# gnns4hri/3D_multi_pose_estimator

Hardware: AMD Instinct MI355X
Metric: frames/sec (5-view Panoptic, 4 persons) at 1/2/4/8 GPUs; MPJPE vs ref (higher is better)
Workload: dtype f32

## Files before the change

3d_multi_pose_estimator_amd/csrc/api.hip:

```cpp
#include <cmath>
#include <cstdarg>
#include <new>
#include <cstdio>
#include <cstdlib>
#include <cstring>

#include "mpe_internal.h"

using namespace mpe;

namespace {

int fail(mpe_ctx *ctx, int code, const char *fmt, ...) {
    char buf[512];
    va_list ap;
    va_start(ap, fmt);
    vsnprintf(buf, sizeof buf, fmt, ap);
    va_end(ap);
    if (ctx) ctx->err = buf;
    return code;
}

#define HIPCHK(ctx, expr)                                                                     \
    do {                                                                                      \
// ... 467 lines not shown
        if (g.in_dim > 512) return false;
    }
    const size_t shm = (size_t)2 * ((size_t)16 * (ctx->cfg.max_heads_per_frame + 1) + (ctx->cfg.max_heads_per_frame + 1) + 1 +
                                    (size_t)(ctx->cfg.n_cameras + 1) * (ctx->cfg.n_cameras + 1)) * sizeof(float);
    return shm <= 40 * 1024;
}

int ensure_lat_workspace(mpe_ctx *ctx) {
    if (ctx->gat_pl[0]) return MPE_OK;
    ctx->lat_rows = ctx->max_nodes < LAT_MAX_NODES ? ctx->max_nodes : LAT_MAX_NODES;
    ctx->gat_pl_plane = (size_t)ctx->lat_rows * ctx->act_ld;
    int rc;
    for (int i = 0; i < 2; ++i)
        if ((rc = dev_alloc(ctx, &ctx->gat_pl[i], 3 * ctx->gat_pl_plane))) return rc;
    return MPE_OK;
}

struct LatTail {
    bool deferred = false;
    const float *ft2 = nullptr;
    int ld = 0;
    float alpha = 0.f, out_slope = 0.f;
    int out_mode = 0;
};

int run_gat_lat(mpe_ctx *ctx, hipStream_t s, const mpe_batch *b, float *d_scores_en, float *d_scores_heads, LatTail *tail = nullptr) {
    if (tail) tail->deferred = false;
    int rc = ensure_lat_workspace(ctx);
    if (rc) return rc;
    const int V = ctx->cfg.n_cameras, J = ctx->cfg.n_joints, hmax = ctx->cfg.max_heads_per_frame;
    const int n_nodes = b->n_heads + b->n_edge_nodes;
    if (n_nodes > ctx->lat_rows) return fail(ctx, MPE_ERR_CAPACITY, "latency path: %d nodes exceed %d", n_nodes, ctx->lat_rows);
    GatLayer &g0 = ctx->gat[0];
    uint16_t *head_src = getenv("MPE_NO_HEAD_SRC_TABLE") ? nullptr : ctx->head_src;
    {
        GemmProf gp(ctx, s, 2.0 * b->n_heads * (double)g0.in_dim * (J * 10), 0, 0);
        HIPCHK(ctx, launch_lat_l0a(s, ctx->d_cfg, *b, V, J, ctx->node_off, ctx->head_frame, ctx->en_frame, ctx->en_pair, ctx->head_src, hmax,
                                   ctx->d_status, ctx->l0_w, (long)weight_rows(g0.in_dim) * ctx->l0_ld, ctx->l0_ld, ctx->l0_b, g0.in_dim, ctx->h0,
                                   ctx->feat_ld, ctx->gat_alpha));
    }
    bool done = false;
    if ((rc = gat_linear(ctx, s, ctx->h0, ctx->feat_ld, g0.fc2, ctx->act[1], ctx->act_ld, b->n_heads, nullptr, false, 0.f, false, nullptr, nullptr,
                         -1.0, nullptr, &done)))
        return rc;
    const int L = ctx->gat_layers;
    for (int l = 0; l < L; ++l) {
// ... 41 lines not shown
            a.ld_out = 1;
            if (tail && coef && !d_scores_heads && g.heads == 1 && g.out_dim == 1) {
                tail->deferred = true;
                tail->ft2 = a.ft2;
                tail->ld = a.ld;
                tail->alpha = a.alpha;
                tail->out_slope = a.out_slope;
                tail->out_mode = a.out_mode;
                return MPE_OK;
            }
        } else {
            a.out_mode = 0;
            a.out = nullptr;
            a.out_pl = ctx->gat_pl[0];
            a.out_pl_plane = ctx->gat_pl_plane;
            a.ld_out = ctx->act_ld;
        }
        HIPCHK(ctx, launch_lat_attention(s, *b, V, hmax, ctx->node_off, ctx->head_frame, ctx->en_frame, ctx->en_pair, a, head_src));
    }
    return MPE_OK;
}

int run_gat(mpe_ctx *ctx, hipStream_t s, const mpe_batch *b, float *d_scores_en, float *d_scores_heads,
            const float *d_feats = nullptr, int ld_feats = 0) {
    int rc = ensure_gat_workspace(ctx);
    if (rc) return rc;
    if (lat_gat_ok(ctx, b, d_feats != nullptr)) return run_gat_lat(ctx, s, b, d_scores_en, d_scores_heads);
    const int V = ctx->cfg.n_cameras, J = ctx->cfg.n_joints;
    const int n_nodes = b->n_heads + b->n_edge_nodes;
    if ((rc = gat_topology(ctx, s, b))) return rc;
    const bool dense_in = d_feats != nullptr;
    if (dense_in) {
        if (ld_feats < ctx->gat[0].in_dim) return fail(ctx, MPE_ERR_INVALID, "feature stride too small");
        if (!ctx->xdense) {
            int rc2 = dev_alloc(ctx, &ctx->xdense, (size_t)ctx->max_nodes * ctx->feat_ld);
            if (rc2) return rc2;
            if ((rc2 = dev_alloc(ctx, &ctx->hdense, (size_t)ctx->max_nodes * ctx->feat_ld))) return rc2;
        }
        HIPCHK(ctx, hipMemcpy2DAsync(ctx->xdense, (size_t)ctx->feat_ld * sizeof(float), d_feats,
                                     (size_t)ld_feats * sizeof(float), (size_t)ctx->gat[0].in_dim * sizeof(float),
                                     n_nodes, hipMemcpyDeviceToDevice, s));
    } else if (ctx->l0_grouped) {
        HIPCHK(ctx, launch_head_features(s, ctx->d_cfg, *b, J, ctx->xc, ctx->l0_ld, 0, 0, false, ctx->cam_count, V));
        HIPCHK(ctx, launch_group_heads(s, b->n_heads, V, b->d_head_cam, ctx->cam_count, ctx->cam_list,
                                       ctx->cfg.max_heads, true));
    } else {
        HIPCHK(ctx, launch_head_features(s, ctx->d_cfg, *b, J, ctx->x0, ctx->feat_ld, 0, 0, true));
    }
    const int L = ctx->gat_layers;
    for (int l = 0; l < L; ++l) {
        const bool last = l == L - 1;
        AggArgs a = gat_agg_args(ctx, l);
        int n_rows_ft2 = 0;
        if ((rc = gat_layer_linear(ctx, s, b, l, l > 0 ? GAT_IN_ACT : dense_in ? GAT_IN_DENSE0 : GAT_IN_IMPLICIT, &a,
                                   &n_rows_ft2)))
            return rc;
        if (last) {
            a.out_mode = ctx->gat_out_mode;
            a.score_mode = 1;
            a.out = d_scores_en;
            a.out_heads = d_scores_heads;
            a.ld_out = 1;
        } else {
            a.out_mode = 0;
            a.out = ctx->act[0];
            a.ld_out = ctx->act_ld;
        }
        if ((rc = gat_attention(ctx, s, b, l, a, n_rows_ft2))) return rc;
    }
    return MPE_OK;
}

int copy_rows_in(mpe_ctx *ctx, hipStream_t s, float *dst, int ld_dst, const float *src, int ld_src, int cols, int rows) {
    if (rows <= 0) return MPE_OK;
    HIPCHK(ctx, hipMemsetAsync(dst, 0, (size_t)rows * ld_dst * sizeof(float), s));
    HIPCHK(ctx, hipMemcpy2DAsync(dst, (size_t)ld_dst * sizeof(float), src, (size_t)ld_src * sizeof(float),
                                 (size_t)cols * sizeof(float), rows, hipMemcpyDeviceToDevice, s));
    return MPE_OK;
}

}

extern "C" {

const char *mpe_version(void) { return "mpe-hip 0.1 (gfx950)"; }
// ... 419 lines not shown
    if ((rc = ensure_gat_workspace(ctx))) return rc;
    for (int k = 0; k < 2; ++k)
        if (ctx->pair_key[k] == b->d_xy) ctx->pair_key[k] = nullptr;
    if (lat_gat_ok(ctx, b, false) && lat_tail_available(hmax, ctx->cl_keys_per_frame) && b->n_edge_nodes > 0) {
        LatTail tail;
        if ((rc = run_gat_lat(ctx, s, b, scores, nullptr, &tail))) return rc;
        if (tail.deferred) {
            const int J = ctx->cfg.n_joints;
            const int slot = ctx->pair_next;
            const size_t need = (size_t)LAT_MAX_FRAMES * hmax * hmax * J * 3;
            const bool pairs_ok = (size_t)b->n_heads <= (size_t)LAT_MAX_FRAMES * hmax;
            if (pairs_ok && !ctx->pair_pts[slot] && (rc = dev_alloc(ctx, &ctx->pair_pts[slot], need, false))) return rc;
            for (int k = 0; k < 2; ++k)
                if (k == slot || ctx->pair_key[k] == b->d_xy) ctx->pair_key[k] = nullptr;
            HIPCHK(ctx, launch_lat_tail(s, ctx->d_cfg, *b, J, ctx->en_pair, ctx->en_frame, tail.ft2, tail.ld, ctx->a12, tail.alpha, tail.out_slope,
                                        tail.out_mode, ctx->node_off, scores, ctx->cfg.max_persons_per_frame, hmax, ctx->cl_keys_per_frame, d_persons,
                                        d_n_persons, pairs_ok ? ctx->pair_pts[slot] : nullptr));
            if (pairs_ok) {
                ctx->pair_key[slot] = b->d_xy;
                ctx->pair_heads[slot] = b->n_heads;
                ctx->pair_en[slot] = b->n_edge_nodes;
                ctx->pair_next = slot ^ 1;
            }
            return MPE_OK;
        }
    } else if ((rc = run_gat(ctx, s, b, scores, nullptr))) {
        return rc;
    }
    HIPCHK(ctx, launch_cluster(s, ctx->d_cfg, *b, ctx->en_pair, scores, ctx->cfg.max_persons_per_frame,
                               ctx->cfg.max_heads_per_frame, ctx->cl_keys, ctx->cl_keys_per_frame, ctx->cl_scratch,
                               ctx->cl_scratch_per_frame, d_persons, d_n_persons));
    return MPE_OK;
}

int mpe_mlp_input_rows(mpe_ctx *ctx, void *stream, const mpe_batch *b, const int32_t *d_persons,
                       const int32_t *d_n_persons, float *d_rows, int32_t ld_rows, uint8_t *d_valid) {
    int rc = check_batch(ctx, b);
    if (rc) return rc;
    if (b->n_frames == 0) return MPE_OK;
    DeviceGuard dg(ctx);
    const int width = ctx->cfg.n_cameras * ctx->cfg.n_joints * ctx->cfg.numbers_per_joint;
    if (!d_persons || !d_n_persons || !d_rows || ld_rows < width)
        return fail(ctx, MPE_ERR_INVALID, "mpe_mlp_input_rows: bad argument");
    HIPCHK(ctx, launch_mlp_rows(static_cast<hipStream_t>(stream), ctx->d_cfg, ctx->cfg.n_cameras, ctx->cfg.n_joints, *b,
                                d_persons, d_n_persons, nullptr, ctx->cfg.max_persons_per_frame, d_rows, ld_rows,
                                d_valid));
    return MPE_OK;
}

static int mlp_chain(mpe_ctx *ctx, hipStream_t s, const float *x, int ld_x, int m, const int32_t *d_m, float **y_out,
                     int *ld_y, const DecodeEpi *dec = nullptr, bool *dec_done = nullptr) {
    if (dec_done) *dec_done = false;
    const float *in = x;
    int ld_in = ld_x;
    int rc;
    for (int l = 0; l < ctx->mlp_layers; ++l) {
// ... 286 lines not shown
```

3d_multi_pose_estimator_amd/csrc/cluster.hip:

```cpp
#include <cstdlib>
#include <cstring>

#include "mpe_internal.h"
#include "dlt_common.h"

namespace mpe {

namespace {

struct PySet {
    int32_t *tab;
    int32_t *alt;
    int mask, fill;
};

__device__ inline int pyset_probe(const int32_t *tab, int mask, int key, bool stop_on_equal, bool *found) {
    unsigned perturb = (unsigned)key;
    int i = key & mask;
    *found = false;
    while (true) {
        int probes = (i + 9 <= mask) ? 9 : 0;
        int j = i;
        while (true) {
            const int cur = tab[j];
// ... 291 lines not shown
            for (int t = lane; t < n / 2; t += 64) {
                const int i = ((t & ~(j - 1)) << 1) | (t & (j - 1));
                const int p = i | j;
                const bool up = (i & k) == 0;
                const uint64_t x = s_keys[i], y = s_keys[p];
                if ((x > y) == up) {
                    s_keys[i] = y;
                    s_keys[p] = x;
                }
            }
            __syncthreads();
        }
    if (lane != 0) return;
    Work w = carve(s_work, hmax, table_cap);
    auto pair_of = [&](int m, int &h1, int &h2) {
        const uint32_t pr = s_pair[m];
        h1 = (int)(pr >> 16);
        h2 = (int)(pr & 0xFFFFu);
    };
    n_persons[f] = greedy_and_components(w, s_keys, n, pair_of, H, M, s_cam, V, cfg->min_views, pcap, out);
}

#define MPE_RL(v, i) __builtin_amdgcn_readlane((int)(v), (i))
__device__ inline int wl(int old, int val, int idx) { return (int)threadIdx.x == idx ? val : old; }

struct RegSet {
    int t0, t1;
    int mask, fill;
};

__device__ inline int rs_get(const RegSet &s, int j) { return j < 64 ? MPE_RL(s.t0, j) : MPE_RL(s.t1, j - 64); }

__device__ inline void rs_put(RegSet &s, int j, int key) {
    if (j < 64) s.t0 = wl(s.t0, key, j);
    else s.t1 = wl(s.t1, key, j - 64);
}

__device__ inline int rs_probe(const RegSet &s, int key, bool stop_on_equal, bool *found) {
    unsigned perturb = (unsigned)key;
    int i = key & s.mask;
    *found = false;
    while (true) {
        int probes = (i + 9 <= s.mask) ? 9 : 0;
        int j = i;
        while (true) {
            const int cur = rs_get(s, j);
            if (cur == -1) return j;
// ... 16 lines not shown
    if (found) return false;
    rs_put(s, j, key);
    s.fill++;
    if (s.fill * 5 < s.mask * 3) return true;
    const int minused = s.fill * 4;
    int newsize = 8;
    while (newsize <= minused) newsize <<= 1;
    RegSet n{-1, -1, newsize - 1, s.fill};
    for (int half = 0; half < 2; ++half) {
        const int t = half ? s.t1 : s.t0;
        unsigned long long bits = __ballot(t != -1);
        while (bits) {
            const int i = __builtin_ctzll(bits);
            bits &= bits - 1;
            bool f2;
            const int k = MPE_RL(t, i);
            rs_put(n, rs_probe(n, k, false, &f2), k);
        }
    }
    s = n;
    return true;
}

__device__ __forceinline__ void cluster_wave_body(uint64_t *s_keys, int f, const DevCfg *__restrict__ cfg, int n_frames,
                                                  const int32_t *__restrict__ head_off, const int32_t *__restrict__ en_off,
                                                  const int32_t *__restrict__ head_cam, const int32_t *__restrict__ en_pair,
                                                  const float *__restrict__ scores, int pcap, int n_pow2, int hmax,
                                                  int32_t *__restrict__ persons, int32_t *__restrict__ n_persons) {
    if (f >= n_frames) return;
    const int V = cfg->V;
    const int lane = threadIdx.x;
    const int h0 = head_off[f], H = head_off[f + 1] - h0;
    const int e0 = en_off[f], M = en_off[f + 1] - e0;
    int32_t *out = persons + (size_t)f * pcap * V;
    if (M <= 0 || H > 64 || H > hmax || M > n_pow2) {
        for (int i = lane; i < pcap * V; i += 64) out[i] = -1;
        if (lane == 0) n_persons[f] = 0;
        return;
    }
    uint32_t *s_pair = reinterpret_cast<uint32_t *>(s_keys + n_pow2);
    const float thr = cfg->threshold;
    const int min_views = cfg->min_views;
    int n_valid = 0;
    for (int m0 = 0; m0 < M; m0 += 64) {
        const int m = m0 + lane;
        uint64_t key = KEY_NONE;
        if (m < M) {
            const int h1 = en_pair[2 * (size_t)(e0 + m)], h2 = en_pair[2 * (size_t)(e0 + m) + 1];
            s_pair[m] = ((uint32_t)h1 << 16) | (uint32_t)h2;
            key = make_key(scores[e0 + m], thr, m);
        }
        const unsigned long long live = __ballot(key != KEY_NONE);
        if (key != KEY_NONE) s_keys[n_valid + __popcll(live & ((1ull << lane) - 1ull))] = key;
        n_valid += __popcll(live);
    }
    int n = 64;
    while (n < n_valid) n <<= 1;
    for (int m = n_valid + lane; m < n; m += 64) s_keys[m] = KEY_NONE;
    __syncthreads();
    for (int k = 2; k <= n; k <<= 1)
        for (int j = k >> 1; j > 0; j >>= 1) {
            for (int t = lane; t < n / 2; t += 64) {
                const int i = ((t & ~(j - 1)) << 1) | (t & (j - 1));
                const int p = i | j;
                const bool up = (i & k) == 0;
                const uint64_t x = s_keys[i], y = s_keys[p];
                if ((x > y) == up) {
                    s_keys[i] = y;
                    s_keys[p] = x;
                }
            }
            __syncthreads();
        }

    int32_t *s_aux = reinterpret_cast<int32_t *>(s_pair + n_pow2);
    int32_t *s_first = s_aux, *s_ord = s_aux + 64, *s_gor = s_aux + 128, *s_gcnt = s_aux + 192;
    const int camv = lane < H ? head_cam[h0 + lane] : 0;
    int linkedv = (int)(1u << camv);
    int humanv = -1, cfhv = 0, eav = -1, ebv = -1;

    s_first[lane] = 0x7FFFFFFF;
    s_gor[lane] = 0;
    s_gcnt[lane] = 0;
    __syncthreads();
    for (int m = lane; m < M; m += 64) {
        const uint32_t pr = s_pair[m];
        atomicMin(&s_first[pr >> 16], 2 * m);
        atomicMin(&s_first[pr & 0xFFFFu], 2 * m + 1);
    }
    __syncthreads();
    const int firstv = s_first[lane];
    const int n_nodes = __popcll(__ballot(firstv != 0x7FFFFFFF));
    {
        int rank = 0;
        for (int l = 0; l < H; ++l) rank += MPE_RL(firstv, l) < firstv ? 1 : 0;
        if (firstv != 0x7FFFFFFF) s_ord[rank] = lane;
    }
    __syncthreads();
    const int orderv = lane < n_nodes ? s_ord[lane] : 0;

    int cur = 0, ne = 0;
    for (int k0 = 0; k0 < n; k0 += 64) {
        const uint64_t key = s_keys[k0 + lane];
        const bool valid = key != KEY_NONE;
        const uint32_t pr = valid ? s_pair[(uint32_t)key] : 0u;
        const int h1 = (int)(pr >> 16), h2 = (int)(pr & 0xFFFFu);
        const bool first1 = pair_first_is_h1(h1, h2);
        const int a_l = first1 ? h1 : h2, b_l = first1 ? h2 : h1;
        const uint32_t ba_l = 1u << __shfl(camv, a_l), bb_l = 1u << __shfl(camv, b_l);
        const int cnt = __popcll(__ballot(valid));
        int start = 0;
        while (true) {
            const uint32_t la_l = (uint32_t)__shfl(linkedv, a_l), lb_l = (uint32_t)__shfl(linkedv, b_l);
            const int ha_l = __shfl(humanv, a_l), hb_l = __shfl(humanv, b_l);
            const uint32_t ca_x = (uint32_t)__shfl(cfhv, ha_l >= 0 ? ha_l : 0);
            const uint32_t cb_x = (uint32_t)__shfl(cfhv, hb_l >= 0 ? hb_l : 0);
            const uint32_t ca_l = ha_l >= 0 ? ca_x : 0u, cb_l = hb_l >= 0 ? cb_x : 0u;
            const bool rej = (lb_l & ba_l) || (la_l & bb_l) || (ca_l & bb_l) || (cb_l & ba_l) ||
                             (ha_l >= 0 && hb_l >= 0 && (cb_l & ca_l));
            const unsigned long long pass = __ballot(valid && lane >= start && !rej);
            if (!pass) break;
// ... 13 lines not shown
                cfhv = wl(cfhv, (int)(ca | bb), ha);
            } else if (hb >= 0 && ha < 0) {
                humanv = wl(humanv, hb, a);
                cfhv = wl(cfhv, (int)(cb | ba), hb);
            } else {
                humanv = humanv == hb ? ha : humanv;
            }
            eav = wl(eav, a, ne);
            ebv = wl(ebv, b, ne);
            ++ne;
            linkedv = wl(linkedv, (int)(la | bb), a);
            linkedv = wl(linkedv, (int)(lb | ba), b);
            start = q + 1;
        }
        if (cnt < 64) break;
    }

    if (humanv >= 0) {
        atomicOr(&s_gor[humanv], 1 << camv);
        atomicAdd(&s_gcnt[humanv], 1);
    }
    for (int i = lane; i < pcap * V; i += 64) out[i] = -1;
    __threadfence_block();
    __syncthreads();
    const bool plainv = __popc((unsigned)s_gor[lane]) == s_gcnt[lane];
    unsigned long long done = 0;
    int np = 0;
    for (int oi = 0; oi < n_nodes; ++oi) {
        const int v = MPE_RL(orderv, oi);
        if ((done >> v) & 1ull) continue;
        const int g = MPE_RL(humanv, v);
        if (g < 0 || MPE_RL((int)plainv, g)) {
            const unsigned long long memb = g >= 0 ? __ballot(humanv == g) : (1ull << v);
            done |= memb;
            if (__popcll(memb) >= min_views && np < pcap) {
                if ((memb >> lane) & 1ull) out[(size_t)np * V + camv] = lane;
                ++np;
            }
            continue;
        }
        RegSet set{-1, -1, 7, 0};
        rs_add(set, v);
        int lvlv = 0, nxtv = 0;
        lvlv = wl(lvlv, v, 0);
        int nl = 1;
        bool full = set.fill == n_nodes;
        while (nl > 0 && !full) {
// ... 39 lines not shown
    if (lane == 0) n_persons[f] = np;
}

__global__ __launch_bounds__(64) void k_cluster_wave(const DevCfg *__restrict__ cfg, int n_frames,
                                                     const int32_t *__restrict__ head_off,
                                                     const int32_t *__restrict__ en_off,
                                                     const int32_t *__restrict__ head_cam,
                                                     const int32_t *__restrict__ en_pair,
                                                     const float *__restrict__ scores, int pcap, int n_pow2,
                                                     int hmax, int32_t *__restrict__ persons,
                                                     int32_t *__restrict__ n_persons) {
    extern __shared__ uint64_t s_keys[];
    cluster_wave_body(s_keys, blockIdx.x, cfg, n_frames, head_off, en_off, head_cam, en_pair, scores, pcap, n_pow2, hmax, persons, n_persons);
}

struct TailScores {
    const float *ft2;
    int ld;
    const float *a12;
    float alpha, out_slope;
    int out_mode;
    const int32_t *node_off;
    float *scores;
};

__global__ __launch_bounds__(256) void k_lat_tail(const DevCfg *__restrict__ cfg, int n_frames, int n_en, int J,
                                                  const int32_t *__restrict__ head_off, const int32_t *__restrict__ en_off,
                                                  const int32_t *__restrict__ head_cam, const int32_t *__restrict__ en_pair,
                                                  const int32_t *__restrict__ en_frame, TailScores ts, int pcap, int n_pow2, int hmax,
                                                  int32_t *__restrict__ persons, int32_t *__restrict__ n_persons,
                                                  const uint32_t *__restrict__ tri_mask, const double *__restrict__ xy,
                                                  double *__restrict__ pair_pts) {
#pragma clang fp contract(off)
    extern __shared__ uint64_t s_keys[];
    if ((int)blockIdx.x < n_frames) {
        if (threadIdx.x >= 64) return;
        const int f = blockIdx.x, lane = threadIdx.x;
        const int hb = head_off[f], H = head_off[f + 1] - hb;
        const int e0 = en_off[f], M = en_off[f + 1] - e0;
        const int nb = ts.node_off[f];
        for (int m = lane; m < M; m += 64) {
            const int h1 = en_pair[2 * (size_t)(e0 + m)], h2 = en_pair[2 * (size_t)(e0 + m) + 1], v = H + m;
            const float *ra1 = ts.a12 + (size_t)(nb + h1) * 32, *ra2 = ts.a12 + (size_t)(nb + h2) * 32, *ra3 = ts.a12 + (size_t)(nb + v) * 32;
            const float a2v = ra3[16];
            float e1 = ra1[0] + a2v, e2 = ra2[0] + a2v, e3 = ra3[0] + a2v;
            e1 = e1 > 0.f ? e1 : e1 * ts.alpha;
            e2 = e2 > 0.f ? e2 : e2 * ts.alpha;
            e3 = e3 > 0.f ? e3 : e3 * ts.alpha;
            const float mx = fmaxf(fmaxf(e1, e2), e3);
            const float x1 = expf(e1 - mx), x2 = expf(e2 - mx), x3 = expf(e3 - mx);
            const float sum = (x1 + x2) + x3;
            const float w1 = x1 / sum, w2 = x2 / sum, w3 = x3 / sum;
            const float v1 = ts.ft2[(size_t)(nb + h1) * ts.ld], v2 = ts.ft2[(size_t)(nb + h2) * ts.ld], v3 = ts.ft2[(size_t)(nb + v) * ts.ld];
            float acc = v1 * w1;
            acc = acc + v2 * w2;
            acc = acc + v3 * w3;
            float o = acc;
            if (ts.out_mode == 0) o = acc > 0.f ? acc : acc * ts.out_slope;
            else if (ts.out_mode == 1) o = 1.f / (1.f + expf(-acc));
            ts.scores[e0 + m] = H > hmax ? 0.f : o;
        }
        __syncthreads();
        cluster_wave_body(s_keys, f, cfg, n_frames, head_off, en_off, head_cam, en_pair, ts.scores, pcap, n_pow2, hmax, persons, n_persons);
        return;
    }
    const size_t i = (size_t)(blockIdx.x - n_frames) * 256 + threadIdx.x;
    if (i >= (size_t)n_en * J) return;
    const int m = (int)(i / J), j = (int)(i - (size_t)m * J);
    const int f = en_frame[m];
    const int hb = head_off[f], H = head_off[f + 1] - hb;
    if (H > hmax) return;
    int la = en_pair[2 * (size_t)m], lb = en_pair[2 * (size_t)m + 1];
    int ca = head_cam[hb + la], cb = head_cam[hb + lb];
    if (ca > cb) {
        const int t = la;
        la = lb;
        lb = t;
        const int c = ca;
        ca = cb;
        cb = c;
    }
    const int ga = hb + la, gb = hb + lb;
    if (!((tri_mask[ga] >> j) & 1u) || !((tri_mask[gb] >> j) & 1u)) return;
    double ua, va, ub, vb;
    dltc::undistort_point(cfg, ca, xy[((size_t)ga * J + j) * 2], xy[((size_t)ga * J + j) * 2 + 1], &ua, &va);
    dltc::undistort_point(cfg, cb, xy[((size_t)gb * J + j) * 2], xy[((size_t)gb * J + j) * 2 + 1], &ub, &vb);
    dltc::dlt_solve(cfg->P[ca], cfg->P[cb], ua, va, ub, vb, pair_pts + (((size_t)ga * hmax + lb) * J + j) * 3);
}

bool lat_tail_available(int hmax, size_t keys_per_frame) {
    if (getenv("MPE_CLUSTER_KERNEL") || hmax > 64) return false;
    int n_pow2 = 64;
    while ((size_t)n_pow2 < keys_per_frame) n_pow2 <<= 1;
    return (size_t)n_pow2 * (sizeof(uint64_t) + sizeof(uint32_t)) + 256 * sizeof(int32_t) <= 48 * 1024;
}

hipError_t launch_lat_tail(hipStream_t s, const DevCfg *cfg, const mpe_batch &b, int J, const int32_t *en_pair, const int32_t *en_frame,
                           const float *ft2, int ld, const float *a12, float alpha, float out_slope, int out_mode, const int32_t *node_off,
                           float *scores, int pcap, int hmax, size_t keys_per_frame, int32_t *persons, int32_t *n_persons, double *pair_pts) {
    if (b.n_frames <= 0) return hipSuccess;
    int n_pow2 = 64;
    while ((size_t)n_pow2 < keys_per_frame) n_pow2 <<= 1;
    const size_t shm = (size_t)n_pow2 * (sizeof(uint64_t) + sizeof(uint32_t)) + 256 * sizeof(int32_t);
    TailScores ts{ft2, ld, a12, alpha, out_slope, out_mode, node_off, scores};
    const size_t items = pair_pts ? (size_t)b.n_edge_nodes * J : 0;
    const unsigned grid = (unsigned)(b.n_frames + (items + 255) / 256);
    hipLaunchKernelGGL(k_lat_tail, dim3(grid), dim3(256), shm, s, cfg, b.n_frames, pair_pts ? b.n_edge_nodes : 0, J, b.d_frame_head_off,
                       b.d_frame_en_off, b.d_head_cam, en_pair, en_frame, ts, pcap, n_pow2, hmax, persons, n_persons, b.d_tri_mask, b.d_xy,
                       pair_pts);
    return hipGetLastError();
}

constexpr int CB_THREADS = 1024;
constexpr int CB_WAVES = CB_THREADS / 64;
constexpr int CB_KCAP = 8192;
constexpr int CB_INF = 0x7FFFFFFF;

__global__ __launch_bounds__(CB_THREADS) void k_cluster_block(const DevCfg *__restrict__ cfg, int n_frames,
                                                              const int32_t *__restrict__ head_off,
                                                              const int32_t *__restrict__ en_off,
                                                              const int32_t *__restrict__ head_cam,
                                                              const int32_t *__restrict__ en_pair,
                                                              const float *__restrict__ scores, int pcap, int hmax,
                                                              int table_cap, uint64_t *__restrict__ keys_all,
                                                              size_t keys_per_frame, int32_t *__restrict__ persons,
                                                              int32_t *__restrict__ n_persons) {
    extern __shared__ uint64_t s_keys[];
    const int f = blockIdx.x;
    if (f >= n_frames) return;
    const int V = cfg->V;
    const int t = threadIdx.x, lane = t & 63, wave = t >> 6;
    const int h0 = head_off[f], H = head_off[f + 1] - h0;
// ... 322 lines not shown
```

3d_multi_pose_estimator_amd/csrc/mpe_internal.h:

```cpp
#pragma once
#include <hip/hip_runtime.h>
#include <stdint.h>
#include <string>
#include <vector>

#include "../../include/mpe.h"

namespace mpe {

constexpr int GEMM_BM = 128;
constexpr int GEMM_BN = 80;
constexpr int GEMM_BK = 32;
constexpr int GEMM_BN_MAX = 208;
inline int weight_rows(int out_dim) { return (out_dim + 15) / 16 * 16 + GEMM_BN_MAX; }
constexpr int LD_ALIGN = 32;

inline int round_up(int x, int m) { return (x + m - 1) / m * m; }

struct Linear {
    float *w = nullptr;
    float *b = nullptr;
    unsigned short *w16 = nullptr;
    int ldw16 = 0;
    unsigned short *w3 = nullptr;
// ... 81 lines not shown
    bool gat_split = true;
    mpe::Linear mlp[MPE_MAX_MLP_LAYERS];
    bool mlp_ready[MPE_MAX_MLP_LAYERS] = {};
    int max_nodes = 0;
    int feat_ld = 0;
    int act_ld = 0;
    float *x0 = nullptr;
    float *h0 = nullptr;
    float *xdense = nullptr;
    float *hdense = nullptr;
    float *xc = nullptr;
    int l0_ld = 0;
    mpe::Linear l0_fc1[MPE_MAX_CAMERAS];
    float *l0_w = nullptr;
    float *l0_b = nullptr;
    int32_t *cam_count = nullptr;
    int32_t *cam_list = nullptr;
    bool l0_grouped = true;
    float *act[3] = {nullptr, nullptr, nullptr};
    float *a12 = nullptr;
    double *pair_pts[2] = {nullptr, nullptr};
    const void *pair_key[2] = {nullptr, nullptr};
    int pair_heads[2] = {0, 0}, pair_en[2] = {0, 0}, pair_next = 0;
    unsigned short *gat_pl[2] = {nullptr, nullptr};
    size_t gat_pl_plane = 0;
    int lat_rows = 0;
    int32_t *head_frame = nullptr;
    int32_t *en_frame = nullptr;
    int32_t *en_pair = nullptr;
    uint16_t *head_src = nullptr;
    size_t head_src_cap = 0;
    int x_m_cap = 0;
    int32_t *node_off = nullptr;
    mpe::ResidualState *res_state = nullptr;
    uint32_t *res_hist = nullptr;
    double *res_partial = nullptr;
    double *log_table = nullptr;
    int n_log = 0;
    uint64_t *cl_keys = nullptr;
    int32_t *cl_scratch = nullptr;
    size_t cl_keys_per_frame = 0, cl_scratch_per_frame = 0;
    int mlp_ld_in = 0, mlp_ld_hidden = 0;
    float *mlp_rows = nullptr;
    float *mlp_act[2] = {nullptr, nullptr};
    int32_t *mlp_count = nullptr;
    float *scores_tmp = nullptr;
// ... 99 lines not shown
                          int32_t *en_frame, int32_t *en_pair, uint16_t *head_src, int hmax, int32_t *status, const float *l0_w,
                          long w_cam_stride, int l0_ld, const float *l0_b, int n_out, float *h0, int ld_h0, float alpha);
hipError_t launch_lat_attention(hipStream_t s, const mpe_batch &b, int V, int max_heads_per_frame, const int32_t *node_off,
                                const int32_t *head_frame, const int32_t *en_frame, const int32_t *en_pair, const AggArgs &a,
                                const uint16_t *head_src);
hipError_t launch_gat_attention(hipStream_t s, const mpe_batch &b, int V, int max_heads_per_frame,
                                const int32_t *node_off, const int32_t *head_frame, const int32_t *en_frame,
                                const int32_t *en_pair, const float *attn_l, const float *attn_r, float *a12,
                                const AggArgs &a, int n_rows_ft2, const uint16_t *head_src, int x_deg_cap = 0,
                                int x_m_cap = 0);

size_t cluster_keys_per_frame(int max_heads_per_frame);
size_t cluster_scratch_per_frame(int max_heads_per_frame);
hipError_t launch_cluster(hipStream_t s, const DevCfg *cfg, const mpe_batch &b, const int32_t *en_pair,
                          const float *scores, int pcap, int max_heads_per_frame, uint64_t *keys,
                          size_t keys_per_frame, int32_t *scratch, size_t scratch_per_frame,
                          int32_t *persons, int32_t *n_persons);

bool lat_tail_available(int hmax, size_t keys_per_frame);
hipError_t launch_lat_tail(hipStream_t s, const DevCfg *cfg, const mpe_batch &b, int J, const int32_t *en_pair, const int32_t *en_frame,
                           const float *ft2, int ld, const float *a12, float alpha, float out_slope, int out_mode, const int32_t *node_off,
                           float *scores, int pcap, int hmax, size_t keys_per_frame, int32_t *persons, int32_t *n_persons, double *pair_pts);

hipError_t launch_person_scan(hipStream_t s, int n_frames, int pcap, const int32_t *n_persons, int32_t *person_off,
                              int32_t *total);
hipError_t launch_mlp_rows(hipStream_t s, const DevCfg *cfg, int V, int J, const mpe_batch &b,
                           const int32_t *persons, const int32_t *n_persons, const int32_t *person_off, int pcap,
                           float *rows, int ld_rows, uint8_t *valid, int32_t *scan_out = nullptr, int32_t *total_out = nullptr,
                           float *zero_poses = nullptr, int n_out = 0, const double *pair_pts = nullptr, int pair_hmax = 0);

hipError_t launch_triangulate(hipStream_t s, const DevCfg *cfg, int V, int J, const mpe_batch &b,
                              const int32_t *persons, const int32_t *n_persons, int pcap, double *poses,
                              uint8_t *joint_valid, uint32_t out_mask, bool positive_ids_only = false);
hipError_t launch_dlt_pairs(hipStream_t s, const DevCfg *cfg, const double *pts, const int32_t *cams, int n,
                            double *out);
hipError_t launch_decode(hipStream_t s, int n_frames, int pcap, int n_out, float scale, const int32_t *n_persons,
                         const int32_t *person_off, const float *y, int ld_y, float *poses);
int cluster_table_cap(int hmax);

hipError_t launch_eval(hipStream_t s, const mpe_eval_args &a);

hipError_t launch_reproject(hipStream_t s, const DevCfg *cfg, int V, const mpe_batch &b, const mpe_reproject_args &a);
hipError_t launch_partition_labels(hipStream_t s, int V, const mpe_batch &b, const mpe_partition_labels_args &a);
hipError_t launch_group_bodies(hipStream_t s, const mpe_group_bodies_args &a);
hipError_t launch_partition_scores(hipStream_t s, const mpe_partition_scores_args &a, const double *log_table, int n_log);
hipError_t launch_residual_stats(hipStream_t s, int V, const mpe_residual_stats_args &a, ResidualState *state, uint32_t *hist,
// ... 4 lines not shown
```

3d_multi_pose_estimator_amd/lib.py:

```python
import ctypes as C
import os

_HERE = os.path.dirname(os.path.abspath(__file__))
LIB_PATH = os.path.join(_HERE, 'libmpe_hip.so')
if os.environ.get('MPE_LIB_VARIANT'):
    LIB_PATH = os.path.join(_HERE, 'libmpe_hip_%s.so' % os.environ['MPE_LIB_VARIANT'])

if os.environ.get('MPE_SET_HW_QUEUES', '0') == '1':
    os.environ.setdefault('GPU_MAX_HW_QUEUES', '8')

MPE_MAX_CAMERAS = 32
MPE_MAX_JOINTS = 32
MPE_ERR_UNSUPPORTED = -6

c_f32p = C.POINTER(C.c_float)
c_f64p = C.POINTER(C.c_double)
c_i32p = C.POINTER(C.c_int32)
c_u32p = C.POINTER(C.c_uint32)
c_u8p = C.POINTER(C.c_uint8)


class MpeError(RuntimeError):
    def __init__(self, code, msg):
        super().__init__('libmpe_hip error %d: %s' % (code, msg))
# ... 89 lines not shown
                ('d_gt_xyz', C.c_void_p), ('d_gt_joint', C.c_void_p), ('d_gt_valid', C.c_void_p), ('d_n_gt_in', C.c_void_p)]


MPE_GT_KEY_SLOTS, MPE_GT_M1_SLOT = 32, 31

MPE_PART_SKIPPED, MPE_PART_OVER_CAP = 1, 2
MPE_PART_MAX_SAMPLES, MPE_PART_MAX_SKELETONS, MPE_PART_MAX_KEYS = 256, 1024, 32

MPE_EVAL_SKIPPED, MPE_EVAL_OVER_CAP, MPE_EVAL_OVER_BUDGET, MPE_EVAL_NO_ASSIGNMENT = 1, 2, 4, 8


SYMBOLS = {
    'mpe_create': (C.c_int, [C.POINTER(mpe_config), C.POINTER(C.c_void_p)]),
    'mpe_destroy': (None, [C.c_void_p]),
    'mpe_last_error': (C.c_char_p, [C.c_void_p]),
    'mpe_version': (C.c_char_p, []),
    'mpe_set_gat_params': (C.c_int, [C.c_void_p, C.c_int32, C.c_float, C.c_float]),
    'mpe_set_gat_layer': (C.c_int, [C.c_void_p, C.c_int32, C.c_int32, C.c_int32, C.c_int32,
                                    c_f32p, c_f32p, c_f32p, c_f32p, c_f32p, c_f32p]),
    'mpe_set_mlp_params': (C.c_int, [C.c_void_p, C.c_int32, C.c_float]),
    'mpe_set_mlp_layer': (C.c_int, [C.c_void_p, C.c_int32, C.c_int32, C.c_int32, c_f32p, c_f32p]),
    'mpe_set_precision': (C.c_int, [C.c_void_p, C.c_int32, C.c_int32]),
    'mpe_match_batch': (C.c_int, [C.c_void_p, C.c_void_p, C.POINTER(mpe_batch), C.c_void_p, C.c_void_p, C.c_void_p]),
    'mpe_mlp3d_batch': (C.c_int, [C.c_void_p, C.c_void_p, C.POINTER(mpe_batch), C.c_void_p, C.c_void_p,
                                  C.c_void_p, C.c_void_p]),
    'mpe_triangulate_batch': (C.c_int, [C.c_void_p, C.c_void_p, C.POINTER(mpe_batch), C.c_void_p, C.c_void_p,
                                        C.c_void_p, C.c_void_p, C.c_uint32]),
    'mpe_upload_linear': (C.c_int, [C.c_void_p, c_f32p, c_f32p, C.c_int32, C.c_int32,
                                    C.POINTER(C.c_void_p), C.POINTER(C.c_void_p), C.POINTER(C.c_int32)]),
    'mpe_free_device': (C.c_int, [C.c_void_p, C.c_void_p]),
    'mpe_linear': (C.c_int, [C.c_void_p, C.c_void_p, C.c_void_p, C.c_int32, C.c_void_p, C.c_int32, C.c_void_p,
                             C.c_void_p, C.c_int32, C.c_int32, C.c_void_p, C.c_int32, C.c_int32, C.c_int32,
                             C.c_float]),
    'mpe_head_features': (C.c_int, [C.c_void_p, C.c_void_p, C.POINTER(mpe_batch), C.c_void_p]),
    'mpe_dense_rows': (C.c_int, [C.c_void_p, C.c_void_p, C.POINTER(mpe_batch), C.c_void_p, C.c_int32]),
    'mpe_gat_forward': (C.c_int, [C.c_void_p, C.c_void_p, C.POINTER(mpe_batch), C.c_void_p, C.c_int32, C.c_void_p,
                                  C.c_void_p]),
    'mpe_set_gat_output': (C.c_int, [C.c_void_p, C.c_int32]),
    'mpe_gat_layer': (C.c_int, [C.c_void_p, C.c_void_p, C.POINTER(mpe_batch), C.c_int32, C.c_void_p, C.c_int32,
                                C.c_void_p, C.c_int32, C.c_int32]),
    'mpe_edge_softmax_aggregate': (C.c_int, [C.c_void_p, C.c_void_p, C.POINTER(mpe_batch), C.c_int32, C.c_void_p,
                                             C.c_int32, C.c_void_p, C.c_int32]),
    'mpe_sync_status': (C.c_int, [C.c_void_p, C.c_void_p]),
    'mpe_status_queue': (C.c_int, [C.c_void_p, C.c_void_p]),
    'mpe_status_wait': (C.c_int, [C.c_void_p, C.c_void_p]),
    'mpe_set_threshold': (C.c_int, [C.c_void_p, C.c_float]),
# ... 93 lines not shown
```

include/mpe.h:

```cpp
#ifndef MPE_H
#define MPE_H

#include <stddef.h>
#include <stdint.h>

#ifdef __cplusplus
extern "C" {
#endif

#define MPE_MAX_CAMERAS 32
#define MPE_MAX_JOINTS 32
#define MPE_MAX_GAT_LAYERS 8
#define MPE_MAX_MLP_LAYERS 16

typedef enum {
    MPE_OK = 0,
    MPE_ERR_INVALID = -1,
    MPE_ERR_CAPACITY = -2,
    MPE_ERR_STATE = -3,
    MPE_ERR_HIP = -4,
    MPE_ERR_NOMEM = -5,
    MPE_ERR_UNSUPPORTED = -6
} mpe_status;

// ... 173 lines not shown

int mpe_head_features(mpe_ctx *ctx, void *stream, const mpe_batch *b, float *d_feat);
int mpe_dense_rows(mpe_ctx *ctx, void *stream, const mpe_batch *b, float *d_rows, int32_t ld);

int mpe_gat_forward(mpe_ctx *ctx, void *stream, const mpe_batch *b, const float *d_feats, int32_t ld_feats,
                    float *d_scores_en, float *d_scores_heads);
int mpe_set_gat_output(mpe_ctx *ctx, int32_t mode);

int mpe_gat_layer(mpe_ctx *ctx, void *stream, const mpe_batch *b, int32_t layer, const float *d_in, int32_t ld_in,
                  float *d_out, int32_t ld_out, int32_t activation);

int mpe_edge_softmax_aggregate(mpe_ctx *ctx, void *stream, const mpe_batch *b, int32_t layer, const float *d_ft2,
                               int32_t ld_ft2, float *d_out, int32_t ld_out);

int mpe_sync_status(mpe_ctx *ctx, void *stream);
int mpe_status_queue(mpe_ctx *ctx, void *stream);
int mpe_status_wait(mpe_ctx *ctx, void *stream);

int mpe_set_threshold(mpe_ctx *ctx, float threshold);

int mpe_cluster_batch(mpe_ctx *ctx, void *stream, const mpe_batch *b, const float *d_scores,
                      int32_t *d_persons, int32_t *d_n_persons);

int mpe_mlp_input_rows(mpe_ctx *ctx, void *stream, const mpe_batch *b, const int32_t *d_persons,
                       const int32_t *d_n_persons, float *d_rows, int32_t ld_rows, uint8_t *d_valid);
int mpe_mlp_forward(mpe_ctx *ctx, void *stream, const float *d_x, int32_t ld_x, int32_t m,
                    float *d_y, int32_t ld_y);

int mpe_dlt_pairs(mpe_ctx *ctx, void *stream, const double *d_pts, const int32_t *d_cams,
                  int32_t n, double *d_out);

typedef struct mpe_packed mpe_packed;
typedef struct {
    int32_t n_frames, n_heads, n_edge_nodes, n_cameras, n_joints;
    const int32_t *frame_head_off, *frame_en_off, *slot_cam, *slot_n, *head_cam, *skeleton_index;
    const uint32_t *joint_mask, *tri_mask;
    const double *xy;
    const float *vp;
} mpe_packed_arrays;
int mpe_pack_json(const char *json, size_t len, const char *const *camera_names, int32_t n_cameras,
                  int32_t n_joints, int32_t frame_start, int32_t frame_step, int32_t max_frames,
                  int32_t n_threads, mpe_packed **out);
int mpe_packed_view(const mpe_packed *pk, mpe_packed_arrays *view);
typedef struct {
    int32_t max_frames, max_heads;
    int32_t *frame_head_off, *frame_en_off, *slot_cam, *slot_n, *head_cam, *skeleton_index;
// ... 90 lines not shown
```

Before: 273,200.

## Fuse final GAT attention with clustering in a multi-wave batch tail kernel

```diff
diff --git a/3d_multi_pose_estimator_amd/csrc/api.hip b/3d_multi_pose_estimator_amd/csrc/api.hip
--- a/3d_multi_pose_estimator_amd/csrc/api.hip
+++ b/3d_multi_pose_estimator_amd/csrc/api.hip
@@ -513,6 +513,8 @@
     int ld = 0;
     float alpha = 0.f, out_slope = 0.f;
     int out_mode = 0;
+    int a12_ready = 1;
+    const float *attn_l = nullptr, *attn_r = nullptr;
 };
 
 int run_gat_lat(mpe_ctx *ctx, hipStream_t s, const mpe_batch *b, float *d_scores_en, float *d_scores_heads, LatTail *tail = nullptr) {
@@ -600,7 +602,8 @@
 }
 
 int run_gat(mpe_ctx *ctx, hipStream_t s, const mpe_batch *b, float *d_scores_en, float *d_scores_heads,
-            const float *d_feats = nullptr, int ld_feats = 0) {
+            const float *d_feats = nullptr, int ld_feats = 0, LatTail *tail = nullptr) {
+    if (tail) tail->deferred = false;
     int rc = ensure_gat_workspace(ctx);
     if (rc) return rc;
     if (lat_gat_ok(ctx, b, d_feats != nullptr)) return run_gat_lat(ctx, s, b, d_scores_en, d_scores_heads);
@@ -639,6 +642,20 @@
             a.out = d_scores_en;
             a.out_heads = d_scores_heads;
             a.ld_out = 1;
+            const GatLayer &g = ctx->gat[l];
+            if (tail && !d_scores_heads && g.heads == 1 && g.out_dim == 1 && !a.ft_half && !b->d_en_pair && n_rows_ft2 == n_nodes &&
+                !getenv("MPE_NO_FUSED_ATTENTION")) {
+                tail->deferred = true;
+                tail->ft2 = a.ft2;
+                tail->ld = a.ld;
+                tail->alpha = a.alpha;
+                tail->out_slope = a.out_slope;
+                tail->out_mode = a.out_mode;
+                tail->a12_ready = a.a12_ready;
+                tail->attn_l = g.attn_l;
+                tail->attn_r = g.attn_r;
+                return MPE_OK;
+            }
         } else {
             a.out_mode = 0;
             a.out = ctx->act[0];
@@ -1104,16 +1121,29 @@
                 ctx->pair_en[slot] = b->n_edge_nodes;
                 ctx->pair_next = slot ^ 1;
             }
+            ctx->match_route = 1;
             return MPE_OK;
         }
-    } else if ((rc = run_gat(ctx, s, b, scores, nullptr))) {
-        return rc;
-    }
+    } else {
+        LatTail tail;
+        const bool want_tail = !getenv("MPE_NO_BATCH_TAIL") && b->n_edge_nodes > 0 && batch_tail_waves(hmax, ctx->cl_keys_per_frame) > 0;
+        if ((rc = run_gat(ctx, s, b, scores, nullptr, nullptr, 0, want_tail ? &tail : nullptr))) return rc;
+        if (tail.deferred) {
+            HIPCHK(ctx, launch_batch_tail(s, ctx->d_cfg, *b, ctx->en_pair, tail.ft2, tail.ld, ctx->a12, tail.a12_ready, tail.attn_l, tail.attn_r,
+                                          tail.alpha, tail.out_slope, tail.out_mode, ctx->node_off, scores, ctx->cfg.max_persons_per_frame, hmax,
+                                          ctx->cl_keys_per_frame, d_persons, d_n_persons));
+            ctx->match_route = 2;
+            return MPE_OK;
+        }
+    }
+    ctx->match_route = 0;
     HIPCHK(ctx, launch_cluster(s, ctx->d_cfg, *b, ctx->en_pair, scores, ctx->cfg.max_persons_per_frame,
                                ctx->cfg.max_heads_per_frame, ctx->cl_keys, ctx->cl_keys_per_frame, ctx->cl_scratch,
                                ctx->cl_scratch_per_frame, d_persons, d_n_persons));
     return MPE_OK;
 }
+
+int mpe_match_route(const mpe_ctx *ctx) { return ctx ? ctx->match_route : -1; }
 
 int mpe_mlp_input_rows(mpe_ctx *ctx, void *stream, const mpe_batch *b, const int32_t *d_persons,
                        const int32_t *d_n_persons, float *d_rows, int32_t ld_rows, uint8_t *d_valid) {
diff --git a/3d_multi_pose_estimator_amd/csrc/cluster.hip b/3d_multi_pose_estimator_amd/csrc/cluster.hip
--- a/3d_multi_pose_estimator_amd/csrc/cluster.hip
+++ b/3d_multi_pose_estimator_amd/csrc/cluster.hip
@@ -337,7 +337,7 @@
 }
 
 #define MPE_RL(v, i) __builtin_amdgcn_readlane((int)(v), (i))
-__device__ inline int wl(int old, int val, int idx) { return (int)threadIdx.x == idx ? val : old; }
+__device__ inline int wl(int old, int val, int idx) { return (int)(threadIdx.x & 63) == idx ? val : old; }
 
 struct RegSet {
     int t0, t1;
@@ -400,6 +400,12 @@
     return true;
 }
 
+__device__ __forceinline__ void wave_sync() {
+    __builtin_amdgcn_fence(__ATOMIC_RELEASE, "workgroup");
+    __builtin_amdgcn_wave_barrier();
+    __builtin_amdgcn_fence(__ATOMIC_ACQUIRE, "workgroup");
+}
+
 __device__ __forceinline__ void cluster_wave_body(uint64_t *s_keys, int f, const DevCfg *__restrict__ cfg, int n_frames,
                                                   const int32_t *__restrict__ head_off, const int32_t *__restrict__ en_off,
                                                   const int32_t *__restrict__ head_cam, const int32_t *__restrict__ en_pair,
@@ -407,7 +413,7 @@
                                                   int32_t *__restrict__ persons, int32_t *__restrict__ n_persons) {
     if (f >= n_frames) return;
     const int V = cfg->V;
-    const int lane = threadIdx.x;
+    const int lane = threadIdx.x & 63;
     const int h0 = head_off[f], H = head_off[f + 1] - h0;
     const int e0 = en_off[f], M = en_off[f + 1] - e0;
     int32_t *out = persons + (size_t)f * pcap * V;
@@ -435,7 +441,7 @@
     int n = 64;
     while (n < n_valid) n <<= 1;
     for (int m = n_valid + lane; m < n; m += 64) s_keys[m] = KEY_NONE;
-    __syncthreads();
+    wave_sync();
     for (int k = 2; k <= n; k <<= 1)
         for (int j = k >> 1; j > 0; j >>= 1) {
             for (int t = lane; t < n / 2; t += 64) {
@@ -448,7 +454,7 @@
                     s_keys[p] = x;
                 }
             }
-            __syncthreads();
+            wave_sync();
         }
 
     int32_t *s_aux = reinterpret_cast<int32_t *>(s_pair + n_pow2);
@@ -460,13 +466,13 @@
     s_first[lane] = 0x7FFFFFFF;
     s_gor[lane] = 0;
     s_gcnt[lane] = 0;
-    __syncthreads();
+    wave_sync();
     for (int m = lane; m < M; m += 64) {
         const uint32_t pr = s_pair[m];
         atomicMin(&s_first[pr >> 16], 2 * m);
         atomicMin(&s_first[pr & 0xFFFFu], 2 * m + 1);
     }
-    __syncthreads();
+    wave_sync();
     const int firstv = s_first[lane];
     const int n_nodes = __popcll(__ballot(firstv != 0x7FFFFFFF));
     {
@@ -474,7 +480,7 @@
         for (int l = 0; l < H; ++l) rank += MPE_RL(firstv, l) < firstv ? 1 : 0;
         if (firstv != 0x7FFFFFFF) s_ord[rank] = lane;
     }
-    __syncthreads();
+    wave_sync();
     const int orderv = lane < n_nodes ? s_ord[lane] : 0;
 
     int cur = 0, ne = 0;
@@ -534,7 +540,7 @@
     }
     for (int i = lane; i < pcap * V; i += 64) out[i] = -1;
     __threadfence_block();
-    __syncthreads();
+    wave_sync();
     const bool plainv = __popc((unsigned)s_gor[lane]) == s_gcnt[lane];
     unsigned long long done = 0;
     int np = 0;
@@ -620,7 +626,50 @@
     int out_mode;
     const int32_t *node_off;
     float *scores;
+    int a12_ready;
+    const float *attn_l, *attn_r;
 };
+
+__device__ __forceinline__ void tail_scores_wave(const TailScores &ts, int f, int lane, const int32_t *__restrict__ head_off,
+                                                 const int32_t *__restrict__ en_off, const int32_t *__restrict__ en_pair, int hmax) {
+#pragma clang fp contract(off)
+    const int hb = head_off[f], H = head_off[f + 1] - hb;
+    const int e0 = en_off[f], M = en_off[f + 1] - e0;
+    const int nb = ts.node_off[f];
+    for (int m = lane; m < M; m += 64) {
+        const int h1 = en_pair[2 * (size_t)(e0 + m)], h2 = en_pair[2 * (size_t)(e0 + m) + 1], v = H + m;
+        const float v1 = ts.ft2[(size_t)(nb + h1) * ts.ld], v2 = ts.ft2[(size_t)(nb + h2) * ts.ld], v3 = ts.ft2[(size_t)(nb + v) * ts.ld];
+        float c1, c2, c3, a2v;
+        if (ts.a12_ready) {
+            const float *ra1 = ts.a12 + (size_t)(nb + h1) * 32, *ra2 = ts.a12 + (size_t)(nb + h2) * 32, *ra3 = ts.a12 + (size_t)(nb + v) * 32;
+            a2v = ra3[16];
+            c1 = ra1[0];
+            c2 = ra2[0];
+            c3 = ra3[0];
+        } else {
+            const float al = ts.attn_l[0], ar = ts.attn_r[0];
+            a2v = __builtin_fmaf(v3, ar, 0.f);
+            c1 = __builtin_fmaf(v1, al, 0.f);
+            c2 = __builtin_fmaf(v2, al, 0.f);
+            c3 = __builtin_fmaf(v3, al, 0.f);
+        }
+        float e1 = c1 + a2v, e2 = c2 + a2v, e3 = c3 + a2v;
+        e1 = e1 > 0.f ? e1 : e1 * ts.alpha;
+        e2 = e2 > 0.f ? e2 : e2 * ts.alpha;
+        e3 = e3 > 0.f ? e3 : e3 * ts.alpha;
+        const float mx = fmaxf(fmaxf(e1, e2), e3);
+        const float x1 = expf(e1 - mx), x2 = expf(e2 - mx), x3 = expf(e3 - mx);
+        const float sum = (x1 + x2) + x3;
+        const float w1 = x1 / sum, w2 = x2 / sum, w3 = x3 / sum;
+        float acc = v1 * w1;
+        acc = acc + v2 * w2;
+        acc = acc + v3 * w3;
+        float o = acc;
+        if (ts.out_mode == 0) o = acc > 0.f ? acc : acc * ts.out_slope;
+        else if (ts.out_mode == 1) o = 1.f / (1.f + expf(-acc));
+        ts.scores[e0 + m] = H > hmax ? 0.f : o;
+    }
+}
 
 __global__ __launch_bounds__(256) void k_lat_tail(const DevCfg *__restrict__ cfg, int n_frames, int n_en, int J,
                                                   const int32_t *__restrict__ head_off, const int32_t *__restrict__ en_off,
@@ -633,32 +682,9 @@
     extern __shared__ uint64_t s_keys[];
     if ((int)blockIdx.x < n_frames) {
         if (threadIdx.x >= 64) return;
-        const int f = blockIdx.x, lane = threadIdx.x;
-        const int hb = head_off[f], H = head_off[f + 1] - hb;
-        const int e0 = en_off[f], M = en_off[f + 1] - e0;
-        const int nb = ts.node_off[f];
-        for (int m = lane; m < M; m += 64) {
-            const int h1 = en_pair[2 * (size_t)(e0 + m)], h2 = en_pair[2 * (size_t)(e0 + m) + 1], v = H + m;
-            const float *ra1 = ts.a12 + (size_t)(nb + h1) * 32, *ra2 = ts.a12 + (size_t)(nb + h2) * 32, *ra3 = ts.a12 + (size_t)(nb + v) * 32;
-            const float a2v = ra3[16];
-            float e1 = ra1[0] + a2v, e2 = ra2[0] + a2v, e3 = ra3[0] + a2v;
-            e1 = e1 > 0.f ? e1 : e1 * ts.alpha;
-            e2 = e2 > 0.f ? e2 : e2 * ts.alpha;
-            e3 = e3 > 0.f ? e3 : e3 * ts.alpha;
-            const float mx = fmaxf(fmaxf(e1, e2), e3);
-            const float x1 = expf(e1 - mx), x2 = expf(e2 - mx), x3 = expf(e3 - mx);
-            const float sum = (x1 + x2) + x3;
-            const float w1 = x1 / sum, w2 = x2 / sum, w3 = x3 / sum;
-            const float v1 = ts.ft2[(size_t)(nb + h1) * ts.ld], v2 = ts.ft2[(size_t)(nb + h2) * ts.ld], v3 = ts.ft2[(size_t)(nb + v) * ts.ld];
-            float acc = v1 * w1;
-            acc = acc + v2 * w2;
-            acc = acc + v3 * w3;
-            float o = acc;
-            if (ts.out_mode == 0) o = acc > 0.f ? acc : acc * ts.out_slope;
-            else if (ts.out_mode == 1) o = 1.f / (1.f + expf(-acc));
-            ts.scores[e0 + m] = H > hmax ? 0.f : o;
-        }
-        __syncthreads();
+        const int f = blockIdx.x;
+        tail_scores_wave(ts, f, threadIdx.x, head_off, en_off, en_pair, hmax);
+        wave_sync();
         cluster_wave_body(s_keys, f, cfg, n_frames, head_off, en_off, head_cam, en_pair, ts.scores, pcap, n_pow2, hmax, persons, n_persons);
         return;
     }
@@ -700,12 +726,61 @@
     int n_pow2 = 64;
     while ((size_t)n_pow2 < keys_per_frame) n_pow2 <<= 1;
     const size_t shm = (size_t)n_pow2 * (sizeof(uint64_t) + sizeof(uint32_t)) + 256 * sizeof(int32_t);
-    TailScores ts{ft2, ld, a12, alpha, out_slope, out_mode, node_off, scores};
+    TailScores ts{ft2, ld, a12, alpha, out_slope, out_mode, node_off, scores, 1, nullptr, nullptr};
     const size_t items = pair_pts ? (size_t)b.n_edge_nodes * J : 0;
     const unsigned grid = (unsigned)(b.n_frames + (items + 255) / 256);
     hipLaunchKernelGGL(k_lat_tail, dim3(grid), dim3(256), shm, s, cfg, b.n_frames, pair_pts ? b.n_edge_nodes : 0, J, b.d_frame_head_off,
                        b.d_frame_en_off, b.d_head_cam, en_pair, en_frame, ts, pcap, n_pow2, hmax, persons, n_persons, b.d_tri_mask, b.d_xy,
                        pair_pts);
+    return hipGetLastError();
+}
+
+constexpr int BT_MAX_WAVES = 4;
+
+__global__ __launch_bounds__(64 * BT_MAX_WAVES) void k_batch_tail(const DevCfg *__restrict__ cfg, int n_frames,
+                                                                  const int32_t *__restrict__ head_off, const int32_t *__restrict__ en_off,
+                                                                  const int32_t *__restrict__ head_cam, const int32_t *__restrict__ en_pair,
+                                                                  TailScores ts, int pcap, int n_pow2, int hmax, int slice_u64,
+                                                                  int32_t *__restrict__ persons, int32_t *__restrict__ n_persons) {
+    extern __shared__ uint64_t s_keys[];
+    const int wave = __builtin_amdgcn_readfirstlane((int)(threadIdx.x >> 6));
+    const int f = (int)blockIdx.x * (int)(blockDim.x >> 6) + wave;
+    if (f < n_frames) {
+        tail_scores_wave(ts, f, threadIdx.x & 63, head_off, en_off, en_pair, hmax);
+        wave_sync();
+        cluster_wave_body(s_keys + (size_t)wave * slice_u64, f, cfg, n_frames, head_off, en_off, head_cam, en_pair, ts.scores, pcap, n_pow2, hmax,
+                          persons, n_persons);
+    }
+}
+
+static size_t cluster_wave_lds(size_t keys_per_frame, int *n_pow2_out) {
+    int n_pow2 = 64;
+    while ((size_t)n_pow2 < keys_per_frame) n_pow2 <<= 1;
+    if (n_pow2_out) *n_pow2_out = n_pow2;
+    return (size_t)n_pow2 * (sizeof(uint64_t) + sizeof(uint32_t)) + 256 * sizeof(int32_t);
+}
+
+int batch_tail_waves(int hmax, size_t keys_per_frame) {
+    if (getenv("MPE_CLUSTER_KERNEL") || hmax > 64) return 0;
+    const size_t per = cluster_wave_lds(keys_per_frame, nullptr);
+    for (int w = BT_MAX_WAVES; w >= 1; w >>= 1)
+        if (w * per <= 64 * 1024) return w;
+    return 0;
+}
+
+hipError_t launch_batch_tail(hipStream_t s, const DevCfg *cfg, const mpe_batch &b, const int32_t *en_pair, const float *ft2, int ld,
+                             const float *a12, int a12_ready, const float *attn_l, const float *attn_r, float alpha, float out_slope,
+                             int out_mode, const int32_t *node_off, float *scores, int pcap, int hmax, size_t keys_per_frame,
+                             int32_t *persons, int32_t *n_persons) {
+    if (b.n_frames <= 0) return hipSuccess;
+    const int waves = batch_tail_waves(hmax, keys_per_frame);
+    if (waves < 1 || (!a12_ready && (!attn_l || !attn_r))) return hipErrorInvalidValue;
+    int n_pow2;
+    const size_t per = cluster_wave_lds(keys_per_frame, &n_pow2);
+    TailScores ts{ft2, ld, a12, alpha, out_slope, out_mode, node_off, scores, a12_ready, attn_l, attn_r};
+    hipLaunchKernelGGL(k_batch_tail, dim3((unsigned)((b.n_frames + waves - 1) / waves)), dim3(64 * waves), waves * per, s, cfg, b.n_frames,
+                       b.d_frame_head_off, b.d_frame_en_off, b.d_head_cam, en_pair, ts, pcap, n_pow2, hmax, (int)(per / sizeof(uint64_t)),
+                       persons, n_persons);
     return hipGetLastError();
 }
 
diff --git a/3d_multi_pose_estimator_amd/csrc/mpe_internal.h b/3d_multi_pose_estimator_amd/csrc/mpe_internal.h
--- a/3d_multi_pose_estimator_amd/csrc/mpe_internal.h
+++ b/3d_multi_pose_estimator_amd/csrc/mpe_internal.h
@@ -127,6 +127,7 @@
     double *pair_pts[2] = {nullptr, nullptr};
     const void *pair_key[2] = {nullptr, nullptr};
     int pair_heads[2] = {0, 0}, pair_en[2] = {0, 0}, pair_next = 0;
+    int match_route = 0;
     unsigned short *gat_pl[2] = {nullptr, nullptr};
     size_t gat_pl_plane = 0;
     int lat_rows = 0;
@@ -272,6 +273,12 @@
                            const float *ft2, int ld, const float *a12, float alpha, float out_slope, int out_mode, const int32_t *node_off,
                            float *scores, int pcap, int hmax, size_t keys_per_frame, int32_t *persons, int32_t *n_persons, double *pair_pts);
 
+int batch_tail_waves(int hmax, size_t keys_per_frame);
+hipError_t launch_batch_tail(hipStream_t s, const DevCfg *cfg, const mpe_batch &b, const int32_t *en_pair, const float *ft2, int ld,
+                             const float *a12, int a12_ready, const float *attn_l, const float *attn_r, float alpha, float out_slope,
+                             int out_mode, const int32_t *node_off, float *scores, int pcap, int hmax, size_t keys_per_frame,
+                             int32_t *persons, int32_t *n_persons);
+
 hipError_t launch_person_scan(hipStream_t s, int n_frames, int pcap, const int32_t *n_persons, int32_t *person_off,
                               int32_t *total);
 hipError_t launch_mlp_rows(hipStream_t s, const DevCfg *cfg, int V, int J, const mpe_batch &b,
diff --git a/3d_multi_pose_estimator_amd/lib.py b/3d_multi_pose_estimator_amd/lib.py
--- a/3d_multi_pose_estimator_amd/lib.py
+++ b/3d_multi_pose_estimator_amd/lib.py
@@ -135,6 +135,7 @@
     'mpe_set_mlp_layer': (C.c_int, [C.c_void_p, C.c_int32, C.c_int32, C.c_int32, c_f32p, c_f32p]),
     'mpe_set_precision': (C.c_int, [C.c_void_p, C.c_int32, C.c_int32]),
     'mpe_match_batch': (C.c_int, [C.c_void_p, C.c_void_p, C.POINTER(mpe_batch), C.c_void_p, C.c_void_p, C.c_void_p]),
+    'mpe_match_route': (C.c_int, [C.c_void_p]),
     'mpe_mlp3d_batch': (C.c_int, [C.c_void_p, C.c_void_p, C.POINTER(mpe_batch), C.c_void_p, C.c_void_p,
                                   C.c_void_p, C.c_void_p]),
     'mpe_triangulate_batch': (C.c_int, [C.c_void_p, C.c_void_p, C.POINTER(mpe_batch), C.c_void_p, C.c_void_p,
diff --git a/include/mpe.h b/include/mpe.h
--- a/include/mpe.h
+++ b/include/mpe.h
@@ -219,6 +219,8 @@
 int mpe_cluster_batch(mpe_ctx *ctx, void *stream, const mpe_batch *b, const float *d_scores,
                       int32_t *d_persons, int32_t *d_n_persons);
 
+int mpe_match_route(const mpe_ctx *ctx);
+
 int mpe_mlp_input_rows(mpe_ctx *ctx, void *stream, const mpe_batch *b, const int32_t *d_persons,
                        const int32_t *d_n_persons, float *d_rows, int32_t ld_rows, uint8_t *d_valid);
 int mpe_mlp_forward(mpe_ctx *ctx, void *stream, const float *d_x, int32_t ld_x, int32_t m,
```

New measurement: 272,800. No clear change (-0.1%).
